# Cjen1/stateright

Measured on AMD Instinct MI355X. Metric: unique states/sec (whole node) + HBM GB/s, 2pc N=9 at 1/2/4/8 MI355X, higher is better.
Workload: dtype u64; 1 GPU; 2pc N=9 spawn_bfs, full check per step (10340352 unique states); model=2pc, rm_count=9, order=fast, parallelism=1 GPU, world_size=1

## Files before the change

stateright_amd/csrc/kernels.hpp:

```cpp
#pragma once
#include <algorithm>
#include <cmath>
#include <cstddef>
#include <cstdlib>

#include "../../include/stateright_gpu.h"
#include "device.hpp"
#include "models.hpp"

namespace sr {

constexpr u64 META_UNSET = ~0ull;
constexpr int META_SHIFT = 44;
constexpr u32 CAND_NONE = 0xffffffffu;
constexpr int MAX_PROBE = 1 << 16;
constexpr int MAX_PROPS = 32;
constexpr int MAX_PARTS = 64;
#ifndef SR_WIDE_PPW_LOG2_MAX
#define SR_WIDE_PPW_LOG2_MAX 5
#endif
#ifndef SR_STAGE_WORDS
#define SR_STAGE_WORDS 1024
#endif
#ifndef SR_DYN_CHUNKS
#define SR_DYN_CHUNKS 1
#endif
constexpr u32 DYN_SHARDS = 8;
#ifndef DYN_MIN_RATIO
#define DYN_MIN_RATIO 6
#endif
#ifndef SR_NARROW_WPB
#define SR_NARROW_WPB 4
#endif
template <class M>
constexpr int expand_wpb() { return M::W >= 4 ? 4 : SR_NARROW_WPB; }
template <class M>
constexpr u32 expand_ppw_log2_max() { return M::W >= 4 ? SR_WIDE_PPW_LOG2_MAX : expand_wpb<M>() >= 8 ? 5 : 6; }
#ifndef SR_WIDE_STAGE_WORDS
#define SR_WIDE_STAGE_WORDS 2048
#endif
#ifndef SR_WIDE_WAVES
#define SR_WIDE_WAVES 3
#endif

enum ErrBits { ERR_TABLE_FULL = 1, ERR_FRONTIER_OVERFLOW = 2, ERR_PEER_TIMEOUT = 4, ERR_EXCHANGE = 8, ERR_DEFERRED = 16,
               ERR_MODEL = 32 };

struct TableView {
    u64* keys;
    u64* meta;
    u64 mask;
    u32 qbits = 0;
    u32 dbits = 0;
    u32 bbits = 0;
    u32 plimit = MAX_PROBE;
    u32 s32 = 0;
};

template <int POL, class T>
__device__ __forceinline__ T probe_load(const T* p);
template <int POL = 0>
__device__ __forceinline__ u64 slot_load(const TableView& t, u64 i) {
    if (t.s32) return (u64)probe_load<POL>(reinterpret_cast<const u32*>(t.keys) + i);
    return probe_load<POL>(t.keys + i);
}
__device__ __forceinline__ u64 slot_cas(const TableView& t, u64 i, u64 tag) {
    if (t.s32) return (u64)atomicCAS(reinterpret_cast<u32*>(t.keys) + i, 0u, (u32)tag);
    return atomicCAS(reinterpret_cast<unsigned long long*>(t.keys + i), 0ull, (unsigned long long)tag);
}
SR_HD u64 table_words(const TableView& t, u64 cap) { return t.s32 ? (cap + 1) / 2 : cap; }

SR_HD u32 encoding_probe_limit(u32 qbits, u32 dbits) {
    return qbits && dbits < 17 ? (1u << dbits) - 2 : (u32)MAX_PROBE;
}

inline double expected_max_displacement(double alpha, double slots) {
    if (alpha <= 0) return 0;
    if (alpha >= 1) return 1e300;
    return std::log(std::max(2.0, slots)) / (alpha - 1.0 - std::log(alpha));
}
inline double max_load_for(u32 plimit, double slots, double cap_load) {
    if (plimit >= (u32)MAX_PROBE) return cap_load;
    double lo = 0.0, hi = cap_load;
    if (expected_max_displacement(hi, slots) <= plimit / 2.0) return hi;
    for (int i = 0; i < 60; ++i) {
        const double mid = 0.5 * (lo + hi);
        (expected_max_displacement(mid, slots) <= plimit / 2.0 ? lo : hi) = mid;
    }
    return lo;
}

struct ProbeKey {
    u64 home;
    u64 tag;
};

using u128 = unsigned __int128;

SR_HD u128 qperm(u128 x, u32 B) {
    const u32 hb = B / 2, ab = B - hb;
    const u64 mb = hb >= 64 ? ~0ull : (1ull << hb) - 1, ma = ab >= 64 ? ~0ull : (1ull << ab) - 1;
    u64 b = (u64)x & mb, a = (u64)(x >> hb) & ma;
    b ^= fmix64(a * 0x9E3779B97F4A7C15ull + 0x2545F4914F6CDD1Dull) & mb;
    a ^= fmix64(b * 0xC2B2AE3D27D4EB4Full + 0x165667B19E3779F9ull) & ma;
    b ^= fmix64(a * 0xD6E8FEB86659FD93ull + 0x94D049BB133111EBull) & mb;
    a ^= fmix64(b * 0xBF58476D1CE4E5B9ull + 0x7F4A7C159E3779B9ull) & ma;
    return ((u128)a << hb) | b;
}

SR_HD u64 qmix(u64 x, u32 B) {
    const u64 m = (1ull << B) - 1;
    const u32 r = (B + 1) / 2;
    x ^= x >> r;
    x = (x * 0xff51afd7ed558ccdull) & m;
    x ^= x >> r;
    x = (x * 0xc4ceb9fe1a85ec53ull) & m;
    x ^= x >> r;
    return x;
}

SR_HD u64 probe_step(const TableView& t) { return t.qbits ? 1ull : 0ull; }
SR_HD ProbeKey fp_probe(const TableView& t, u64 fp) { return ProbeKey{fp & t.mask, fp}; }
SR_HD ProbeKey quot_probe(const TableView& t, u128 h) {
    return ProbeKey{(u64)(h >> t.qbits), (((u64)h & ((1ull << t.qbits) - 1)) << t.dbits) | 1ull};
}
SR_HD u128 quot_decode(const TableView& t, u64 i, u64 v) {
    const u64 d = (v & ((1ull << t.dbits) - 1)) - 1;
    return ((u128)((i - d) & t.mask) << t.qbits) | (v >> t.dbits);
}
SR_HD ProbeKey reprobe(const TableView& from, const TableView& to, u64 i, u64 v) {
    return from.qbits ? quot_probe(to, quot_decode(from, i, v)) : fp_probe(to, v);
}

inline u32 forced_probe_limit() {
    const char* e = std::getenv("SR_DISP_LIMIT");
    return e ? (u32)std::max(1, std::atoi(e)) : 0u;
}
constexpr u32 SLOT32_DMIN = 10;
inline bool slot32_enabled() {
    static const bool on = !std::getenv("SR_SLOT32") || std::atoi(std::getenv("SR_SLOT32")) != 0;
    return on;
}
constexpr u32 QUOT_MAX_REMAINDER = 56;
template <class M>
inline bool quotient_model(const M& m) {
    if constexpr (has_qkey<M>::value) {
        const int B = m.qkey_bits();
        if constexpr (M::W == 1) return B >= 2 && B <= 62;
        else return B >= 2 && B <= 96;
    }
    (void)m;
    return false;
}
template <class M>
inline TableView make_table_view(const M& m, u64* keys, u64* meta, u64 cap, bool natural = false) {
    TableView v{keys, meta, cap - 1};
    if constexpr (has_qkey<M>::value) {
        const u32 B = (u32)m.qkey_bits();
        u32 k = 0;
        while ((1ull << k) < cap) ++k;
        if (quotient_model(m)) {
            v.qbits = B > k ? B - k : 1u;
            v.bbits = B;
            if (v.qbits > QUOT_MAX_REMAINDER)
                throw Error(SR_ERR_ARG, "make_table_view: a quotient table below min_table_cap");
            if (M::W == 1 && slot32_enabled() && v.qbits + SLOT32_DMIN <= 32) {
                v.s32 = 1;
                v.dbits = 32 - v.qbits;
            } else {
                v.dbits = 64 - v.qbits;
            }
        }
    }
    v.plimit = encoding_probe_limit(v.qbits, v.dbits);
    if (!natural && forced_probe_limit()) v.plimit = std::min(v.plimit, forced_probe_limit());
// ... 487 lines not shown
        if constexpr (HAS) {
            u64 c, s;
            m.action_masks(lane, &c, &s);
            clr_lo = (u32)c, clr_hi = (u32)(c >> 32), set_lo = (u32)s, set_hi = (u32)(s >> 32);
        }
    }
    __device__ __forceinline__ u64 next(u64 s, u32 slot) const {
        const int at = (int)(slot << 2);
        const u32 cl = (u32)__builtin_amdgcn_ds_bpermute(at, (int)clr_lo), ch = (u32)__builtin_amdgcn_ds_bpermute(at, (int)clr_hi);
        const u32 sl = (u32)__builtin_amdgcn_ds_bpermute(at, (int)set_lo), sh = (u32)__builtin_amdgcn_ds_bpermute(at, (int)set_hi);
        return (s & ~((u64)ch << 32 | cl)) | ((u64)sh << 32 | sl);
    }
};


template <class M, class P>
__device__ __forceinline__ void wave_append(const M& m, u64 mask, bool nw, const u64* ns, u32 spar, P par,
                                            u64* stage, u32* stage_par, u32 STAGE, u32* stage_n,
                                            u64* __restrict__ next, P* __restrict__ next_par, u32 next_cap,
                                            LevelCounters* lc, u32 undiscovered) {
    constexpr int W = M::W;
    if (!mask) return;
    const int lane = threadIdx.x & 63;
    const u32 cnt = __popcll(mask);
    const u32 below = __popcll(mask & ((1ull << lane) - 1));
    const int leader = __builtin_ctzll(mask);
    u32 sb = 0;
    if (lane == leader) sb = atomicAdd(stage_n, cnt);
    sb = lane_u32(sb, (u32)leader);
    const u32 in_stage = sb >= STAGE ? 0u : min(cnt, STAGE - sb);
    u32 gb = 0;
    if (cnt > in_stage && lane == leader) gb = atomicAdd(&lc->claims, cnt - in_stage);
    gb = lane_u32(gb, (u32)leader);
    if (!nw) return;
    if (below < in_stage) {
        const u32 kk = sb + below;
#pragma unroll
        for (int x = 0; x < W; ++x) stage[kk * W + x] = ns[x];
        if (stage_par) stage_par[kk] = spar;
    } else {
        const u32 pos = gb + (below - in_stage);
        if (pos < next_cap) {
            store_state<W>(next, pos, ns);
            next_par[pos] = par;
        } else {
            atomicOr(&lc->err, (u32)ERR_FRONTIER_OVERFLOW);
        }
        eval_props(m, ns, pos, undiscovered, lc);
    }
}

template <int R, bool FP_ONLY>
struct ProbeKeys {
    u64 kh[FP_ONLY ? 1 : R], kt[R];
    u32 vmask = 0;
};
template <int POL, bool STATS, int R, bool FP_ONLY>
__device__ __forceinline__ u32 probe_queue(const TableView& t, ProbeKeys<R, FP_ONLY> k, u32* err,
                                           u32* probes = nullptr, u32* cas = nullptr) {
    u32 vmask = k.vmask;
    u32 nmask = 0;
    u32 st = 0, cr = 0, disp = 0;
    u64 si = 0, tag = 0;
    const u64 step = probe_step(t);
    for (;;) {
        if (st == 0 && vmask) {
            cr = (u32)__builtin_ctz(vmask);
            vmask &= vmask - 1;
            tag = k.kt[0];
#pragma unroll
            for (int r = 1; r < R; ++r)
                if (cr == (u32)r) tag = k.kt[r];
            if constexpr (FP_ONLY) {
                si = tag & t.mask;
            } else {
                si = k.kh[0];
#pragma unroll
                for (int r = 1; r < R; ++r)
                    if (cr == (u32)r) si = k.kh[FP_ONLY ? 0 : r];
            }
            st = 1;
            disp = 0;
        }
        if (!__ballot(st != 0)) break;
        u64 v = 0;
        if (st == 1) v = slot_load<POL>(t, si);
        if (st == 2) v = slot_cas(t, si, tag);
        if constexpr (STATS) {
            *probes += st == 1;
            *cas += st == 2;
        }
        if (st != 0) {
            if (v == tag) {
                st = 0;
            } else if (v == 0) {
                if (st == 2) nmask |= 1u << cr;
                st = st == 1 ? 2u : 0u;
            } else if (++disp >= t.plimit) {
                atomicOr(err, (u32)ERR_TABLE_FULL);
                st = 0;
            } else {
                si = (si + 1) & t.mask;
                tag += step;
                st = 1;
            }
        }
    }
    return nmask;
}

#ifndef SR_TIMELINE
#define SR_TIMELINE 0
#endif
constexpr u32 TL_STAMPS = 16, TL_BLOCKS = 2048, TL_LAUNCHES = 64;
#if SR_TIMELINE
__device__ u64* g_timeline;
#define SR_TL(k)                                                            \
    do {                                                                    \
        if (tl_on) {                                                        \
            asm volatile("s_waitcnt vmcnt(0) lgkmcnt(0)" ::: "memory");     \
            tl_ts[k] = __builtin_amdgcn_s_memrealtime();                    \
        }                                                                   \
    } while (0)
#else
#define SR_TL(k) \
    do {         \
    } while (0)
#endif

template <class M, int PB, int POL, bool STATS = false, bool NOPF = false, bool DYN = false, bool BAL = false>
__global__ void __launch_bounds__(64 * expand_wpb<M>()) __attribute__((amdgpu_waves_per_eu(M::W >= 4 ? SR_WIDE_WAVES : PB < 0 ? 6 : 1))) expand_fast(M m, const u64* __restrict__ frontier, u32 lo, u32 hi,
                                                   TableView t, u64* __restrict__ next, u32* __restrict__ next_par,
                                                   u32 next_cap, LevelCounters* lc, u32 undiscovered,
                                                   HostCounters* hc, u32 seq, u32 reset, u32 ppw_log2,
                                                   u32 filt_log2, SlotWork sw) {
    constexpr int W = M::W, MW = M::MW;
    constexpr int STAGE = W >= 4 ? SR_WIDE_STAGE_WORDS / W : SR_STAGE_WORDS;
    extern __shared__ u64 filt[];
    __shared__ u64 stage[STAGE * W];
    __shared__ u32 stage_par[STAGE];
    constexpr u32 PPW_LOG2_MAX = expand_ppw_log2_max<M>();
    constexpr int WPB = expand_wpb<M>();
    __shared__ u64 pst[WPB][(1 << PPW_LOG2_MAX) * W];
#ifndef SR_MAPCAP
#define SR_MAPCAP 1024
#endif
#ifndef SR_WIDE_MAPCAP
#define SR_WIDE_MAPCAP 256
#endif
    constexpr u32 MAPCAP = W >= 4 ? SR_WIDE_MAPCAP : SR_MAPCAP * 4 / expand_wpb<M>();
    static_assert(MW * 64 <= 1024, "action ids must fit 10 bits");
    __shared__ u16 smap[WPB][MAPCAP];
    __shared__ u32 stage_n, base, scratch[2 * WPB];
    const int lane = threadIdx.x & 63, wid = threadIdx.x >> 6;
    if (threadIdx.x == 0) stage_n = 0;
#if SR_TIMELINE
    const bool tl_on = threadIdx.x == 0 && blockIdx.x < TL_BLOCKS && g_timeline;
    u64 tl_ts[TL_STAMPS];
#pragma unroll
    for (u32 k = 0; k < TL_STAMPS; ++k) tl_ts[k] = 0;
    bool tl_first_chunk = true, tl_first_round = true;
    auto tl_store = [&]() {
        if (!tl_on) return;
        u64* t = g_timeline + ((u64)(seq % TL_LAUNCHES) * TL_BLOCKS + blockIdx.x) * TL_STAMPS;
#pragma unroll
        for (u32 k = 0; k < TL_STAMPS; ++k) t[k] = tl_ts[k];
        t[TL_STAMPS - 1] = (u64)gridDim.x << 32 | (u64)(hi - lo);
    };
#endif
    SR_TL(0);
    const bool svc = sw.pub || sw.zero;
    if (svc && blockIdx.x == gridDim.x - 1) {
        if (threadIdx.x < 64) slot_service<M::NPROPS>(sw, threadIdx.x);
        SR_TL(9);
#if SR_TIMELINE
        tl_store();
#endif
        return;
    }
    const u32 nblk = gridDim.x - (svc ? 1u : 0u);
    const bool tbl = ActionTable<M>::HAS && (sw.flags & SLOT_ACTION_TABLE) != 0;
    ActionTable<M> atab;
    if (tbl) atab.fill(m, lane);
    static_assert(!(DYN && BAL), "dynamic chunks keep the fixed geometry");
    ppw_log2 = min(ppw_log2, PPW_LOG2_MAX);
    constexpr bool balanced = BAL;
    LevelGeom geom = level_geometry(0, nblk, (u32)WPB, 1u << ppw_log2, false);
    const u64 r_spec = geom.wave_first(geom.first_chunk(lo, blockIdx.x), (u32)wid) + lane;
    u64 nxt[W];
    const bool chained = sw.chain != nullptr;
    const bool spec_first = sw.prev_n && !chained && !balanced && lane < (int)geom.pw && r_spec < next_cap;
    if (spec_first) load_state<W>(frontier, r_spec, nxt);
    if (sw.prev_n) {
        const u64 ce = __hip_atomic_load(reinterpret_cast<const u64*>(sw.prev_n), __ATOMIC_RELAXED, __HIP_MEMORY_SCOPE_AGENT);
        u64 fb = sw.fbase, ub = sw.ubase;
        if (chained) {
            fb = __hip_atomic_load(&sw.chain->next_base, __ATOMIC_RELAXED, __HIP_MEMORY_SCOPE_AGENT);
            ub = __hip_atomic_load(&sw.chain->unique, __ATOMIC_RELAXED, __HIP_MEMORY_SCOPE_AGENT);
            frontier = sw.arena + fb * W;
            next = sw.arena + fb * W;
            next_par = sw.apar + fb;
            next_cap = (u32)min(sw.arena_cap > fb ? sw.arena_cap - fb : 0ull, 0xffffffffull);
        }
        u32 nn = (ce >> 32) ? 0u : (u32)ce;
        if (sw.gmul && nn) {
            const u64 grow = ((u64)nn * sw.gmul) >> 8;
            const u64 left = next_cap > nn ? (u64)(next_cap - nn) : 0ull;
            if (ub + nn + grow > sw.room || grow > left) {
                nn = 0;
                if (blockIdx.x == 0 && threadIdx.x == 0) atomicOr(&lc->err, (u32)ERR_DEFERRED);
            }
        }
        hi = lo + nn;
        next += (u64)nn * W;
        next_par += nn;
        next_cap = next_cap > nn ? next_cap - nn : 0u;
        if (sw.arena && blockIdx.x == 0 && threadIdx.x == 0) {
            lc->next_base = fb + nn;
            lc->unique = ub + nn;
        }
    } else if (sw.arena && blockIdx.x == 0 && threadIdx.x == 0) {
        lc->next_base = sw.fbase + (hi - lo);
        lc->unique = sw.ubase + (hi - lo);
    }
    SR_TL(1);
    if (balanced) geom = level_geometry(hi - lo, nblk, (u32)WPB, 1u << ppw_log2, true);
    const u32 ppw = geom.pw;
    const u64 chunk = geom.cw;
    const u64 r_first = geom.wave_first(geom.first_chunk(lo, blockIdx.x), (u32)wid) + lane;
    const bool fcompact = M::W == 1 && has_qkey<M>::value && (filt_log2 & FILT_COMPACT) != 0;
    filt_log2 &= FILT_COMPACT - 1;
    const u32 fmask = filt_log2 ? (1u << filt_log2) - 1 : 0;
    const u32 fwords = !fmask ? 0u : fcompact ? (fmask + 1) / 2 : fmask + 1;
    if (lo + (u64)blockIdx.x * chunk < hi)
        for (u32 i = threadIdx.x; i < fwords; i += blockDim.x) filt[i] = 0;
    auto level = [&](const u64* __restrict__ frontier, u32 lo, u32 hi, u64* __restrict__ next,
                     u32* __restrict__ next_par, u32 next_cap, LevelCounters* lc, u32 undiscovered) {
    u32 succ = 0, enabled = 0, probes = 0, cas = 0;
    const u64 cstride = geom.stride(nblk);
    const u64 c_first = geom.first_chunk(lo, blockIdx.x);
    const u32 lim_first = BAL ? geom.chunk_end(c_first, hi) : hi;
    if (!spec_first && lane < (int)ppw && r_first < lim_first) load_state<W>(frontier, r_first, nxt);
    constexpr bool PF = W < 4 || !NOPF;
    if constexpr (!PF) {
        if (lane < (int)ppw && r_first < lim_first) {
#pragma unroll
            for (int i = 0; i < W; ++i) pst[wid][lane * W + i] = nxt[i];
        }
    }
    const u64 nchunks = hi > lo ? ((u64)hi - lo + chunk - 1) / chunk : 0;
    const bool dyn = DYN && SR_DYN_CHUNKS && nblk >= DYN_SHARDS && nchunks > (u64)DYN_MIN_RATIO * nblk;
    const u32 dshard = blockIdx.x % DYN_SHARDS;
    __shared__ u64 s_cnext;
    u64 c_next = c_first + cstride;
    u32 kpend = 0;
    bool pend = false, first_chunk = true;
    for (u64 c0 = c_first; c0 < hi;) {
        const u32 wave0 = (u32)geom.wave_first(c0, (u32)wid);
        const u32 lim = BAL ? geom.chunk_end(c0, hi) : hi;
        const u32 r = wave0 + lane;
        u32 cnt = 0;
        u64 s[W];
        if constexpr (PF) {
#pragma unroll
            for (int i = 0; i < W; ++i) s[i] = nxt[i];
            const u64 rn = geom.wave_first(c_next, (u32)wid) + lane;
            if (lane < (int)ppw && rn < (BAL ? geom.chunk_end(c_next, hi) : hi)) load_state<W>(frontier, rn, nxt);
        } else if (c0 != c_first && lane < (int)ppw && r < lim) {
            load_state<W>(frontier, r, s);
#pragma unroll
            for (int i = 0; i < W; ++i) pst[wid][lane * W + i] = s[i];
        }
        __syncthreads();
        u64 mk[MW];
#pragma unroll
        for (int i = 0; i < MW; ++i) mk[i] = 0;
        if constexpr (has_enabled_slot<M>::value) {
            static_assert(MW == 1 && M::ESLOTS <= 64 && 64 % M::ESLOTS == 0, "enabled_slot: ESLOTS must divide 64");
            static_assert(!has_self_loops<M>::value, "enabled_slot: no self_loops hook");
            constexpr u32 ES = M::ESLOTS, PPP = 64 / ES;
            if (PF && lane < (int)ppw && r < lim) {
#pragma unroll
                for (int i = 0; i < W; ++i) pst[wid][lane * W + i] = s[i];
            }
            wave_lds_sync();
            const u32 np = lim > wave0 ? min(ppw, lim - wave0) : 0u;
            u64 mine = 0;
            for (u32 p0 = 0; p0 < np; p0 += PPP) {
                const u32 p = p0 + (u32)lane / ES, k = (u32)lane % ES;
                const bool en = p < np && m.enabled_slot(&pst[wid][p * W], (int)k);
                const u64 b = __ballot(en);
                const u32 i = (u32)lane - p0;
                if ((u32)lane >= p0 && i < PPP) mine = ES == 64 ? b : (b >> (i * ES)) & ((1ull << (ES % 64)) - 1);
            }
            if (lane < (int)ppw && r < lim) {
                mk[0] = mine;
                cnt = (u32)__popcll(mine);
            }
#if SR_TIMELINE
            if (tl_first_chunk) SR_TL(2);
            if (tl_first_chunk) SR_TL(10);
#endif
        } else
        if (lane < ppw && r < lim) {
            if constexpr (!PF) {
#pragma unroll
                for (int i = 0; i < W; ++i) s[i] = pst[wid][lane * W + i];
            }
            if constexpr (has_enabled_moves<M>::value) {
                succ += m.enabled_moves(s, mk);
            } else {
                m.enabled(s, mk);
            }
#if SR_TIMELINE
            if (tl_first_chunk) SR_TL(2);
#endif
            if constexpr (has_self_loops<M>::value && !has_enabled_moves<M>::value) {
                u64 sl[MW];
                m.self_loops(s, mk, sl);
#pragma unroll
                for (int i = 0; i < MW; ++i) {
                    succ += __popcll(sl[i]);
                    mk[i] &= ~sl[i];
                }
            }
            if constexpr (PF) {
#pragma unroll
                for (int i = 0; i < W; ++i) pst[wid][lane * W + i] = s[i];
            }
#pragma unroll
            for (int i = 0; i < MW; ++i) cnt += __popcll(mk[i]);
#if SR_TIMELINE
            if (tl_first_chunk) SR_TL(10);
#endif
        }
        const u32 incl = wave_incl_scan(cnt);
        u32 nidx = incl - cnt;
        const u32 total = lane_u32(incl, 63);
        if (lane == 0) enabled += total;
#if SR_TIMELINE
        if (tl_first_chunk) SR_TL(11);
#endif

        auto append_new = [&](bool nw, const u64* ns, u32 par) {
            const u64 mask = __ballot(nw);
            if (!mask) return;
            const u32 cnt = __popcll(mask);
            const u32 below = __popcll(mask & ((1ull << lane) - 1));
            const int leader = __builtin_ctzll(mask);
            u32 sb = 0;
            if (lane == leader) sb = atomicAdd(&stage_n, cnt);
            sb = lane_u32(sb, (u32)leader);
            const u32 in_stage = sb >= (u32)STAGE ? 0u : min(cnt, (u32)STAGE - sb);
            u32 gb = 0;
            if (cnt > in_stage && lane == leader) gb = atomicAdd(&lc->claims, cnt - in_stage);
            gb = lane_u32(gb, (u32)leader);
            if (!nw) return;
            const u32 pr = wave0 + par;
            if (below < in_stage) {
                const u32 kk = sb + below;
#pragma unroll
                for (int x = 0; x < W; ++x) stage[kk * W + x] = ns[x];
                stage_par[kk] = pr;
            } else {
                const u32 pos = gb + (below - in_stage);
                if (pos < next_cap) {
                    store_state<W>(next, pos, ns);
                    next_par[pos] = pr;
                    if (sw.naeb) sw.naeb[pos] = sw.peb[pr];
                } else {
                    atomicOr(&lc->err, (u32)ERR_FRONTIER_OVERFLOW);
                }
                eval_props(m, ns, pos, undiscovered, lc);
            }
        };
        for (u32 w0 = 0; w0 < total; w0 += MAPCAP) {
        const u32 wend = min(total, w0 + MAPCAP);
        if (MW <= 2 && ppw <= 8) {
            const u32 excl = incl - cnt;
            for (u32 j0 = w0; j0 < wend; j0 += 64) {
                const u32 j = j0 + (u32)lane;
                u32 p = 0;
#pragma unroll
                for (int q = 1; q < 8; ++q) {
                    const u32 ex = lane_u32(excl, (u32)q);
                    if ((u32)q < ppw && ex <= j) p = (u32)q;
                }
                const u32 k = j - (u32)__shfl((int)excl, (int)p, 64);
                const u64 m0 = __shfl(mk[0], (int)p, 64);
                const u64 m1 = MW > 1 ? __shfl(mk[MW > 1 ? 1 : 0], (int)p, 64) : 0ull;
                const u32 c0 = (u32)__popcll(m0);
                const u32 a = k < c0 ? select_bit(m0, k) : 64u + select_bit(m1, k - c0);
                if (j < wend) smap[wid][j - w0] = (u16)(p | a << 6);
            }
        } else
        while (nidx < wend && nidx < incl) {
            u32 a = 0;
#pragma unroll
            for (int w = MW - 1; w >= 0; --w)
                if (mk[w]) a = (u32)w * 64 + (u32)__builtin_ctzll(mk[w]);
            mk[a >> 6] &= mk[a >> 6] - 1;
            smap[wid][nidx - w0] = (u16)((u32)lane | a << 6);
            ++nidx;
        }
#if SR_TIMELINE
        if (tl_first_chunk) SR_TL(12);
#endif
        wave_lds_sync();
#if SR_TIMELINE
        if (tl_first_chunk) SR_TL(3);
        tl_first_chunk = false;
#endif

        if constexpr (PB < 0) {
            constexpr int R = -PB;
            constexpr bool FP_ONLY = !has_qkey<M>::value;
            for (u32 s0 = w0; s0 < wend; s0 += 64u * R) {
                u64 kh[FP_ONLY ? 1 : R], kt[R];
                u32 vmask = 0;
#pragma unroll
                for (int r = 0; r < R; ++r) {
                    if (!FP_ONLY) kh[FP_ONLY ? 0 : r] = 0;
                    kt[r] = 0;
                    const u32 i = s0 + (u32)r * 64u + (u32)lane;
                    u32 te = 0;
                    u64 tp = 0, tq = 0;
                    if (tbl) {
                        te = i < wend ? smap[wid][i - w0] : 0u;
                        tp = pst[wid][(te & 63) * W];
                        tq = atab.next(tp, te >> 6);
                    }
                    if (i < wend) {
                        u64 ps[W], q[W];
                        bool ok = true;
                        if (tbl) {
                            ps[0] = tp, q[0] = tq;
                        } else {
                            const u32 e = smap[wid][i - w0];
                            const u32 p = e & 63, a = e >> 6;
#pragma unroll
                            for (int x = 0; x < W; ++x) ps[x] = pst[wid][p * W + x];
                            ok = m.apply(ps, (int)a, q);
                        }
                        if (ok) {
                            ++succ;
                            if constexpr (!exact_moves_model<M>) ok = !same_state<W>(q, ps);
                        }
                        if (ok) {
                            const ProbeKey k = probe_key(m, t, q);
                            if (fmask)
                                ok = !filter_seen(filt, fcompact, filt_log2, fmask, t, filter_key(t, k));
                            if (!FP_ONLY) kh[FP_ONLY ? 0 : r] = k.home;
                            kt[r] = k.tag;
                        }
                        if (ok) vmask |= 1u << r;
                    }
                }
#if SR_TIMELINE
                if (tl_first_round) SR_TL(4);
#endif
                u32 nmask = 0;
                u32 st = 0, cr = 0, disp = 0;
                u64 si = 0, tag = 0;
                const u64 step = probe_step(t);
                for (;;) {
                    if (st == 0 && vmask) {
                        cr = (u32)__builtin_ctz(vmask);
                        vmask &= vmask - 1;
                        tag = kt[0];
#pragma unroll
                        for (int r = 1; r < R; ++r)
                            if (cr == (u32)r) tag = kt[r];
                        if constexpr (FP_ONLY) {
                            si = tag & t.mask;
                        } else {
                            si = kh[0];
#pragma unroll
                            for (int r = 1; r < R; ++r)
                                if (cr == (u32)r) si = kh[FP_ONLY ? 0 : r];
                        }
                        st = 1;
                        disp = 0;
                    }
                    if (!__ballot(st != 0)) break;
                    u64 v = 0;
                    if (st == 1) v = slot_load<POL>(t, si);
                    if (st == 2) v = slot_cas(t, si, tag);
                    if constexpr (STATS) {
                        probes += st == 1;
                        cas += st == 2;
                    }
                    if (st != 0) {
                        if (v == tag) {
                            st = 0;
                        } else if (v == 0) {
                            if (st == 2) nmask |= 1u << cr;
                            st = st == 1 ? 2u : 0u;
                        } else if (++disp >= t.plimit) {
                            atomicOr(&lc->err, (u32)ERR_TABLE_FULL);
                            st = 0;
                        } else {
                            si = (si + 1) & t.mask;
                            tag += step;
                            st = 1;
                        }
                    }
                }
#if SR_TIMELINE
                if (tl_first_round) SR_TL(5);
                tl_first_round = false;
#endif
#pragma unroll
                for (int r = 0; r < R; ++r) {
                    const bool nw = nmask >> r & 1;
                    u64 q[W];
                    u32 p = 0;
                    if (tbl) {
                        if (__ballot(nw)) {
                            const u32 e = nw ? smap[wid][s0 + (u32)r * 64u + (u32)lane - w0] : 0u;
                            p = e & 63;
                            q[0] = atab.next(pst[wid][p * W], e >> 6);
                        }
                    } else if (nw) {
                        const u32 e = smap[wid][s0 + (u32)r * 64u + (u32)lane - w0];
                        p = e & 63;
                        u64 ps[W];
#pragma unroll
                        for (int x = 0; x < W; ++x) ps[x] = pst[wid][p * W + x];
                        m.apply(ps, (int)(e >> 6), q);
                    }
                    append_new(nw, q, p);
                }
            }
        } else
        for (u32 it = w0; it < wend; it += 64 * PB) {
            u64 ns[PB][W], cur[PB];
            ProbeKey pk[PB];
            u32 par[PB];
            bool ok[PB];
#pragma unroll
            for (int j = 0; j < PB; ++j) {
                const u32 i = it + j * 64 + lane;
                ok[j] = i < wend;
                par[j] = 0;
                if (tbl) {
                    const u32 e = ok[j] ? smap[wid][i - w0] : 0u;
                    par[j] = e & 63;
                    const u64 ps0 = pst[wid][par[j] * W];
                    ns[j][0] = atab.next(ps0, e >> 6);
                    if constexpr (!exact_moves_model<M>) {
                        if (ok[j] && ns[j][0] == ps0) {
                            ++succ;
                            ok[j] = false;
                        }
                    }
                } else if (ok[j]) {
                    const u32 e = smap[wid][i - w0];
                    const u32 p = e & 63, a = e >> 6;
                    u64 ps[W];
#pragma unroll
                    for (int x = 0; x < W; ++x) ps[x] = pst[wid][p * W + x];
                    ok[j] = m.apply(ps, (int)a, ns[j]);
                    par[j] = p;
                    if constexpr (!exact_moves_model<M>) {
                        if (ok[j] && same_state<W>(ns[j], ps)) {
                            ++succ;
                            ok[j] = false;
                        }
                    }
                }
                pk[j] = ok[j] ? probe_key(m, t, ns[j]) : ProbeKey{0, 0};
                if (fmask && ok[j]) {
                    if (filter_seen(filt, fcompact, filt_log2, fmask, t, filter_key(t, pk[j]))) {
                        ++succ;
                        ok[j] = false;
                    }
                }
            }
#pragma unroll
            for (int j = 0; j < PB; ++j) {
                cur[j] = ok[j] ? slot_load<POL>(t, pk[j].home) : 0;
                if constexpr (STATS) probes += ok[j];
            }
#if SR_TIMELINE
            if (tl_first_round) SR_TL(4);
#endif
            bool nw[PB];
#pragma unroll
            for (int j = 0; j < PB; ++j) {
                nw[j] = false;
                if (!ok[j]) continue;
                ++succ;
                if (cur[j] == pk[j].tag) continue;
                find_or_claim_from<POL>(t, pk[j], cur[j], &nw[j], &lc->err, STATS ? &probes : nullptr,
                                        STATS ? &cas : nullptr);
            }
#if SR_TIMELINE
            if (tl_first_round) SR_TL(5);
            tl_first_round = false;
#endif
#pragma unroll
            for (int j = 0; j < PB; ++j) {
                const u64 mask = __ballot(nw[j]);
                if (!mask) continue;
                const u32 cnt = __popcll(mask);
                const u32 below = __popcll(mask & ((1ull << lane) - 1));
                const int leader = __builtin_ctzll(mask);
                u32 sb = 0;
                if (lane == leader) sb = atomicAdd(&stage_n, cnt);
                sb = lane_u32(sb, (u32)leader);
                const u32 in_stage = sb >= (u32)STAGE ? 0u : min(cnt, (u32)STAGE - sb);
                u32 gb = 0;
                if (cnt > in_stage && lane == leader) gb = atomicAdd(&lc->claims, cnt - in_stage);
                gb = lane_u32(gb, (u32)leader);
                if (!nw[j]) continue;
                const u32 pr = wave0 + par[j];
                if (below < in_stage) {
                    const u32 kk = sb + below;
#pragma unroll
                    for (int x = 0; x < W; ++x) stage[kk * W + x] = ns[j][x];
                    stage_par[kk] = pr;
                } else {
                    const u32 pos = gb + (below - in_stage);
                    if (pos < next_cap) {
                        store_state<W>(next, pos, ns[j]);
                        next_par[pos] = pr;
                        if (sw.naeb) sw.naeb[pos] = sw.peb[pr];
                    } else {
                        atomicOr(&lc->err, (u32)ERR_FRONTIER_OVERFLOW);
                    }
                    eval_props(m, ns[j], pos, undiscovered, lc);
                }
            }
        }
        wave_lds_sync();
        }
        if (dyn && threadIdx.x == 0) {
            u64 cn = hi;
            if (first_chunk) {
                cn = c_first + 2 * cstride;
            } else if (pend) {
                const u64 k = 3ull * nblk + dshard + (u64)DYN_SHARDS * kpend;
                if (k < nchunks) cn = lo + k * chunk;
            }
            pend = cn < hi;
            if (pend) {
                u32 zoff;
                asm volatile("v_mov_b32 %0, 0" : "=v"(zoff));
                kpend = atomicAdd(&lc->chunk_next[dshard][0] + zoff, 1u);
            }
            s_cnext = cn;
        }
        first_chunk = false;
        __syncthreads();
        c0 = c_next;
        c_next = dyn ? s_cnext : c_next + cstride;
        if (stage_n >= (u32)STAGE / 2) {
            const u32 nst = min(stage_n, (u32)STAGE);
            if (threadIdx.x == 0) base = atomicAdd(&lc->claims, nst);
            __syncthreads();
            for (u32 i = threadIdx.x; i < nst; i += blockDim.x) {
                const u32 pos = base + i;
                u64 ns[W];
#pragma unroll
                for (int x = 0; x < W; ++x) ns[x] = stage[i * W + x];
                if (pos < next_cap) {
                    store_state<W>(next, pos, ns);
                    next_par[pos] = stage_par[i];
                    if (sw.naeb) sw.naeb[pos] = sw.peb[stage_par[i]];
                } else {
                    atomicOr(&lc->err, (u32)ERR_FRONTIER_OVERFLOW);
                }
                eval_props(m, ns, pos, undiscovered, lc);
            }
            __syncthreads();
            if (threadIdx.x == 0) stage_n = 0;
        }
    }
    if (dyn && threadIdx.x == 0 && atomicAdd(&lc->chunk_done, 1u) == nblk - 1) {
#pragma unroll
        for (u32 x = 0; x < DYN_SHARDS; ++x) atomicExch(&lc->chunk_next[x][0], 0u);
        atomicExch(&lc->chunk_done, 0u);
    }
    SR_TL(6);
    const bool repair = (sw.flags & SLOT_REPAIR) != 0;
    __syncthreads();
    const u32 n = min(stage_n, (u32)STAGE);
    u32 my_base = 0;
    if (threadIdx.x == 0 && n) my_base = atomicAdd(&lc->claims, n);
    u32 total_succ, total_enabled;
    block_sum2(repair ? 0u : succ, repair ? 0u : enabled, scratch, total_succ, total_enabled);
    u32 total_probes = STATS ? block_sum(probes, scratch) : 0u;
    u32 total_cas = STATS ? block_sum(cas, scratch) : 0u;
    if (threadIdx.x == 0) {
        base = my_base;
        add_stats(lc, total_succ, total_enabled, total_probes, total_cas);
    }
    SR_TL(7);
    __syncthreads();
    for (u32 i = threadIdx.x; i < n; i += blockDim.x) {
        u32 pos = base + i;
        u64 ns[W];
#pragma unroll
        for (int x = 0; x < W; ++x) ns[x] = stage[i * W + x];
        if (pos < next_cap) {
            store_state<W>(next, pos, ns);
            next_par[pos] = stage_par[i];
            if (sw.naeb) sw.naeb[pos] = sw.peb[stage_par[i]];
        } else {
            atomicOr(&lc->err, (u32)ERR_FRONTIER_OVERFLOW);
        }
        eval_props(m, ns, pos, undiscovered, lc);
    }
    };
    level(frontier, lo, hi, next, next_par, next_cap, lc, undiscovered);
    SR_TL(8);
    if (hc) publish<M::NPROPS>(lc, hc, seq, reset != 0, nullptr);
    SR_TL(9);
#if SR_TIMELINE
    tl_store();
#endif
}

template <class M>
__global__ void __launch_bounds__(256) expand_fifo(M m, const u64* __restrict__ frontier, u32 lo, u32 hi, u32 n,
                                                   TableView t, u32* __restrict__ cand, u32 A, u32 level,
                                                   LevelCounters* lc, HostCounters* hc, u32 seq, u32 count_succ) {
    __shared__ u32 scratch[4];
    const u32 r = lo + blockIdx.x * blockDim.x + threadIdx.x;
    u32 succ = 0, claims = 0;
    if (r < hi) {
        u64 s[M::W];
        load_state<M::W>(frontier, r, s);
        const u64 lvl = (u64)(level + 1) << META_SHIFT;
        for_each_successor(m, s, [&](int a, const u64* ns) {
            succ += count_succ;
            if (same_state<M::W>(ns, s)) return;
            bool is_new;
            u64 slot = find_or_claim(t, probe_key(m, t, ns), &is_new, &lc->err);
            if (slot == ~0ull) return;
            claims += is_new;
            const u64 tag = lvl | ((u64)r * A + (u64)a);
            u64 cur = is_new ? META_UNSET : t.meta[slot];
            if (cur != META_UNSET && (cur >> META_SHIFT) != (u64)(level + 1)) return;
            if (tag < cur) atomicMin(reinterpret_cast<unsigned long long*>(&t.meta[slot]), (unsigned long long)tag);
            cand[(u64)a * n + r] = (u32)slot;
        });
    }
    u32 ts = block_sum(succ, scratch);
    u32 tc = block_sum(claims, scratch);
    if (threadIdx.x == 0) {
        add_stats(lc, ts, 0);
        if (tc) atomicAdd(&lc->claims, tc);
    }
    publish<M::NPROPS>(lc, hc, seq, false, nullptr);
}

template <class M>
__global__ void __launch_bounds__(256) own_count(const u32* __restrict__ cand, u32 n, u32 A, u32 level, TableView t,
                                                 u32* __restrict__ counts) {
    u32 r = blockIdx.x * blockDim.x + threadIdx.x;
    if (r >= n) return;
    const u64 lvl = (u64)(level + 1) << META_SHIFT;
    u32 c = 0;
    for (u32 a = 0; a < A; ++a) {
        u32 slot = cand[(u64)a * n + r];
        if (slot != CAND_NONE && t.meta[slot] == (lvl | ((u64)r * A + a))) ++c;
    }
    counts[r] = c;
}

template <class M>
__device__ __forceinline__ void scatter_fifo_body(M m, const u64* __restrict__ frontier, const u32* __restrict__ cand,
                                                  const u32* __restrict__ offs, u32 n, u32 A, u32 level,
                                                  TableView t, u64* __restrict__ next, u32* __restrict__ next_par,
                                                  LevelCounters* lc, u32 undiscovered,
                                                  const u32* __restrict__ peb = nullptr, u32* __restrict__ next_eb = nullptr) {
    u32 r = blockIdx.x * blockDim.x + threadIdx.x;
    if (r >= n) return;
    const u64 lvl = (u64)(level + 1) << META_SHIFT;
    const u32 eb = peb ? peb[r] : 0u;
    u64 s[M::W];
    bool loaded = false;
    u32 j = offs[r];
    for (u32 a = 0; a < A; ++a) {
        u32 slot = cand[(u64)a * n + r];
        if (slot == CAND_NONE || t.meta[slot] != (lvl | ((u64)r * A + a))) continue;
        if (!loaded) {
            load_state<M::W>(frontier, r, s);
            loaded = true;
        }
        u64 ns[M::W];
        m.apply(s, (int)a, ns);
        store_state<M::W>(next, j, ns);
        next_par[j] = r;
        if (next_eb) next_eb[j] = eb;
        eval_props(m, ns, j, undiscovered, lc);
        ++j;
    }
}

template <class M>
__global__ void __launch_bounds__(256) scatter_fifo(M m, const u64* __restrict__ frontier, const u32* __restrict__ cand,
                                                    const u32* __restrict__ offs, u32 n, u32 A, u32 level,
                                                    TableView t, u64* __restrict__ next, u32* __restrict__ next_par,
                                                    LevelCounters* lc, u32 undiscovered, HostCounters* hc, u32 seq,
                                                    const u32* owners, const u32* peb, u32* next_eb) {
    scatter_fifo_body(m, frontier, cand, offs, n, A, level, t, next, next_par, lc, undiscovered, peb, next_eb);
    publish<M::NPROPS>(lc, hc, seq, true, owners);
}

template <class M>
__global__ void __launch_bounds__(256) ev_scan(M m, const u64* __restrict__ frontier, const u32* __restrict__ eb_in,
                                               u32 n, u32 eund, u32 emask, u32* __restrict__ tsat, u32* evf) {
    const u32 r = blockIdx.x * blockDim.x + threadIdx.x;
    if (r >= n) return;
    u64 s[M::W];
    load_state<M::W>(frontier, r, s);
    bool any = false;
    for_each_successor(m, s, [&](int, const u64*) { any = true; });
    u32 sat = 0;
    for (u32 e = emask; e; e &= e - 1) {
        const int p = __builtin_ctz(e);
        if (m.discovers(p, s)) sat |= 1u << p;
    }
    tsat[r] = sat | (any ? 0u : 0x80000000u);
    if (!any)
        for (u32 c = eb_in[r] & ~sat & eund; c; c &= c - 1) atomicMin(&evf[__builtin_ctz(c)], r);
}

template <int = 0> __global__ void __launch_bounds__(256) ev_resolve(const u32* __restrict__ tsat, const u32* __restrict__ eb_in, u32 limit,
                                                  u32 eund, const u32* __restrict__ evf, u32* __restrict__ peb,
                                                  u32* evl) {
    const u32 r = blockIdx.x * blockDim.x + threadIdx.x;
    if (r >= limit) return;
    const u32 ts = tsat[r], sat = ts & 0x7fffffffu;
    u32 clear = 0;
    for (u32 c = sat & eund; c; c &= c - 1) {
        const int p = __builtin_ctz(c);
        if (r <= evf[p]) clear |= 1u << p;
    }
    const u32 eff = eb_in[r] & ~clear;
    peb[r] = eff;
    if (ts >> 31)
        for (u32 c = eff; c; c &= c - 1) atomicMax(&evl[__builtin_ctz(c)], r + 1);
}

template <int = 0> __global__ void fill_u32(u32* p, u32 n, u32 v) {
    const u32 i = blockIdx.x * blockDim.x + threadIdx.x;
    if (i < n) p[i] = v;
}


template <class M>
__global__ void __launch_bounds__(256) count_successors(M m, const u64* __restrict__ frontier, u32 n, u32* counts) {
    u32 r = blockIdx.x * blockDim.x + threadIdx.x;
    if (r >= n) return;
    u64 s[M::W];
    load_state<M::W>(frontier, r, s);
    u32 c = 0;
    for_each_successor(m, s, [&](int, const u64*) { ++c; });
// ... 262 lines not shown
```

Baseline: 7.018 billion unique states/s.

## Give each wave a private staging region instead of a shared LDS atomic counter

When the model has a single-word state and exact moves, the shared LDS stage buffer is split into per-wave regions. Each wave tracks its fill in a register instead of doing an LDS atomicAdd on stage_n for every ballot. Flush decisions come from per-wave fill words published before the existing barrier, using a headroom flag so a region cannot overflow in the next round. Each wave then flushes its own region without the trailing __syncthreads. This removes LDS atomics and one barrier per flush, at the cost of smaller per-wave capacity, which may send more overflow to global atomics or trigger more frequent flushes.

```diff
diff --git a/stateright_amd/csrc/kernels.hpp b/stateright_amd/csrc/kernels.hpp
--- a/stateright_amd/csrc/kernels.hpp
+++ b/stateright_amd/csrc/kernels.hpp
@@ -21,6 +21,9 @@
 #endif
 #ifndef SR_STAGE_WORDS
 #define SR_STAGE_WORDS 1024
+#endif
+#ifndef SR_STAGE_PER_WAVE
+#define SR_STAGE_PER_WAVE 1
 #endif
 #ifndef SR_DYN_CHUNKS
 #define SR_DYN_CHUNKS 1
@@ -814,8 +817,17 @@
     static_assert(MW * 64 <= 1024, "action ids must fit 10 bits");
     __shared__ u16 smap[WPB][MAPCAP];
     __shared__ u32 stage_n, base, scratch[2 * WPB];
+    constexpr bool REGIONS = SR_STAGE_PER_WAVE && W == 1 &&
+                             (PB > 0 || (has_enabled_moves<M>::value && exact_moves_model<M> && !has_emask<M>::value)) &&
+                             !(is_canon<M>::value && STATS && PB > 0);
+    constexpr u32 REG = (u32)STAGE / (u32)WPB;
+    static_assert(!REGIONS || (REG >= 64 && REG < 65536), "a region holds a round and fits fill's 16 bits");
+    __shared__ __attribute__((aligned(16))) u32 fill[WPB];
+    u32 wfill = 0;
     const int lane = threadIdx.x & 63, wid = threadIdx.x >> 6;
+    const u32 rbase = REGIONS ? lane_u32((u32)wid * REG, 0) : 0u;
     if (threadIdx.x == 0) stage_n = 0;
+    if (REGIONS && threadIdx.x < (u32)WPB) fill[threadIdx.x] = 0;
 #if SR_TIMELINE
     const bool tl_on = threadIdx.x == 0 && blockIdx.x < TL_BLOCKS && g_timeline;
     u64 tl_ts[TL_STAMPS];
@@ -1010,10 +1022,17 @@
             const u32 cnt = __popcll(mask);
             const u32 below = __popcll(mask & ((1ull << lane) - 1));
             const int leader = __builtin_ctzll(mask);
-            u32 sb = 0;
-            if (lane == leader) sb = atomicAdd(&stage_n, cnt);
-            sb = lane_u32(sb, (u32)leader);
-            const u32 in_stage = sb >= (u32)STAGE ? 0u : min(cnt, (u32)STAGE - sb);
+            u32 sb = 0, in_stage;
+            if constexpr (REGIONS) {
+                sb = wfill;
+                in_stage = min(cnt, REG - sb);
+                wfill = sb + in_stage;
+                sb += rbase;
+            } else {
+                if (lane == leader) sb = atomicAdd(&stage_n, cnt);
+                sb = lane_u32(sb, (u32)leader);
+                in_stage = sb >= (u32)STAGE ? 0u : min(cnt, (u32)STAGE - sb);
+            }
             u32 gb = 0;
             if (cnt > in_stage && lane == leader) gb = atomicAdd(&lc->claims, cnt - in_stage);
             gb = lane_u32(gb, (u32)leader);
@@ -1268,10 +1287,17 @@
                 const u32 cnt = __popcll(mask);
                 const u32 below = __popcll(mask & ((1ull << lane) - 1));
                 const int leader = __builtin_ctzll(mask);
-                u32 sb = 0;
-                if (lane == leader) sb = atomicAdd(&stage_n, cnt);
-                sb = lane_u32(sb, (u32)leader);
-                const u32 in_stage = sb >= (u32)STAGE ? 0u : min(cnt, (u32)STAGE - sb);
+                u32 sb = 0, in_stage;
+                if constexpr (REGIONS) {
+                    sb = wfill;
+                    in_stage = min(cnt, REG - sb);
+                    wfill = sb + in_stage;
+                    sb += rbase;
+                } else {
+                    if (lane == leader) sb = atomicAdd(&stage_n, cnt);
+                    sb = lane_u32(sb, (u32)leader);
+                    in_stage = sb >= (u32)STAGE ? 0u : min(cnt, (u32)STAGE - sb);
+                }
                 u32 gb = 0;
                 if (cnt > in_stage && lane == leader) gb = atomicAdd(&lc->claims, cnt - in_stage);
                 gb = lane_u32(gb, (u32)leader);
@@ -1314,29 +1340,58 @@
             s_cnext = cn;
         }
         first_chunk = false;
+        if constexpr (REGIONS) {
+            if (lane == 0) {
+                const u32 d = wfill - (fill[wid] & 0xffffu);
+                fill[wid] = wfill | (wfill + d + d / 4 > REG ? 1u << 16 : 0u);
+            }
+        }
         __syncthreads();
         c0 = c_next;
         c_next = dyn ? s_cnext : c_next + cstride;
-        if (stage_n >= (u32)STAGE / 2) {
-            const u32 nst = min(stage_n, (u32)STAGE);
+        u32 nst, before = 0;
+        bool flush;
+        if constexpr (REGIONS) {
+            u32 flags = 0;
+            nst = 0;
+#pragma unroll
+            for (int w = 0; w < WPB; ++w) {
+                const u32 f = fill[w];
+                if (w < wid) before += f & 0xffffu;
+                nst += f & 0xffffu;
+                flags |= f;
+            }
+            flush = nst && ((flags >> 16) != 0 || nst >= (u32)STAGE / 2);
+        } else {
+            nst = min(stage_n, (u32)STAGE);
+            flush = stage_n >= (u32)STAGE / 2;
+        }
+        if (flush) {
             if (threadIdx.x == 0) base = atomicAdd(&lc->claims, nst);
             __syncthreads();
-            for (u32 i = threadIdx.x; i < nst; i += blockDim.x) {
-                const u32 pos = base + i;
+            const u32 i0 = REGIONS ? (u32)lane : threadIdx.x, i1 = REGIONS ? wfill : nst;
+            for (u32 i = i0; i < i1; i += REGIONS ? 64u : blockDim.x) {
+                const u32 pos = base + before + i;
+                const u32 k = rbase + i;
                 u64 ns[W];
 #pragma unroll
-                for (int x = 0; x < W; ++x) ns[x] = stage[i * W + x];
+                for (int x = 0; x < W; ++x) ns[x] = stage[k * W + x];
                 if (pos < next_cap) {
                     store_state<W>(next, pos, ns);
-                    next_par[pos] = stage_par[i];
-                    if (sw.naeb) sw.naeb[pos] = sw.peb[stage_par[i]];
+                    next_par[pos] = stage_par[k];
+                    if (sw.naeb) sw.naeb[pos] = sw.peb[stage_par[k]];
                 } else {
                     atomicOr(&lc->err, (u32)ERR_FRONTIER_OVERFLOW);
                 }
                 eval_props(m, ns, pos, undiscovered, lc);
             }
-            __syncthreads();
-            if (threadIdx.x == 0) stage_n = 0;
+            if constexpr (REGIONS) {
+                wfill = 0;
+                if (lane == 0) fill[wid] = 0;
+            } else {
+                __syncthreads();
+                if (threadIdx.x == 0) stage_n = 0;
+            }
         }
     }
     if (dyn && threadIdx.x == 0 && atomicAdd(&lc->chunk_done, 1u) == nblk - 1) {
@@ -1347,7 +1402,18 @@
     SR_TL(6);
     const bool repair = (sw.flags & SLOT_REPAIR) != 0;
     __syncthreads();
-    const u32 n = min(stage_n, (u32)STAGE);
+    u32 n, before = 0;
+    if constexpr (REGIONS) {
+        n = 0;
+#pragma unroll
+        for (int w = 0; w < WPB; ++w) {
+            const u32 f = fill[w] & 0xffffu;
+            if (w < wid) before += f;
+            n += f;
+        }
+    } else {
+        n = min(stage_n, (u32)STAGE);
+    }
     u32 my_base = 0;
     if (threadIdx.x == 0 && n) my_base = atomicAdd(&lc->claims, n);
     u32 total_succ, total_enabled;
@@ -1360,15 +1426,17 @@
     }
     SR_TL(7);
     __syncthreads();
-    for (u32 i = threadIdx.x; i < n; i += blockDim.x) {
-        u32 pos = base + i;
+    const u32 i0 = REGIONS ? (u32)lane : threadIdx.x, i1 = REGIONS ? wfill : n;
+    for (u32 i = i0; i < i1; i += REGIONS ? 64u : blockDim.x) {
+        u32 pos = base + before + i;
+        const u32 k = rbase + i;
         u64 ns[W];
 #pragma unroll
-        for (int x = 0; x < W; ++x) ns[x] = stage[i * W + x];
+        for (int x = 0; x < W; ++x) ns[x] = stage[k * W + x];
         if (pos < next_cap) {
             store_state<W>(next, pos, ns);
-            next_par[pos] = stage_par[i];
-            if (sw.naeb) sw.naeb[pos] = sw.peb[stage_par[i]];
+            next_par[pos] = stage_par[k];
+            if (sw.naeb) sw.naeb[pos] = sw.peb[stage_par[k]];
         } else {
             atomicOr(&lc->err, (u32)ERR_FRONTIER_OVERFLOW);
         }
```

New measurement: 7.120 billion unique states/s, median of 6. +1.5%, better.
